# maxgreat/Instance-Search

Hardware: AMD Instinct MI355X
Metric: images/sec descriptor extract + query x gallery search (higher is better)
Workload: dtype f32; 1 GPU; BASELINE configs[1]: ResNet-50 fully-conv global descriptors + top-100 cosine search, 10000-row gallery shard per GPU, 224x224 synthetic images; gallery_rows_per_gpu=10000, descriptor_dim=2048, k=100, backbone=resnet50, backbone_dtype=f32, activation_layout=NHWC, bn_folded=True, parallelism=gallery-row shards x1 + DP extraction, ranks=1

## Files before the change

include/isx.h:

```cpp
#ifndef ISX_H_
#define ISX_H_

#include <stddef.h>
#include <stdint.h>

#ifdef __cplusplus
extern "C" {
#endif

#define ISX_CONV_CHUNK 64

#define ISX_OK 0
#define ISX_ERR_ARG (-1)
#define ISX_ERR_WORKSPACE (-2)
#define ISX_ERR_HIP (-3)

typedef void* isx_stream_t;

const char* isx_last_error(void);
int isx_version(void);


int isx_l2norm_rows(const float* x, int64_t B, int64_t D, float eps, float* y, isx_stream_t stream);

int isx_l2norm_shift_rows(const float* x, const float* shift, int64_t B, int64_t F, float eps, float* y,
                          isx_stream_t stream);

int isx_gap_l2(const float* fmap, int64_t B, int C, int H, int W, float eps, float* y, isx_stream_t stream);

int isx_gap_l2_nhwc(const float* fmap, int64_t B, int C, int H, int W, float eps, float* y, isx_stream_t stream);

int isx_bias_act_inplace(float* y, const float* bias, const float* residual, int64_t n, int C, int64_t inner, int relu,
                         isx_stream_t stream);

int isx_images_u8_to_f32(const uint8_t* img, int64_t B, int H, int W, float mean0, float mean1, float mean2, float std0, float std1,
                         float std2, int channels_last, float* out, isx_stream_t stream);

int isx_bias_relu_maxpool_nhwc(const float* y, const float* bias, int64_t B, int H, int W, int C, float* out, isx_stream_t stream);

int isx_conv3x3_expand_nhwc(const float* x, int64_t B, int H, int W, int Cin, const float* w2_ohwi, const float* b2, int stride,
                            const float* w3t, int Cout, const float* b3, const float* residual, int relu, float* y, isx_stream_t stream);

int isx_conv3x3_expand_dual_nhwc(const float* t, int64_t B, int H, int W, int Cin, const float* w2_ohwi, const float* b2, const float* x2,
                                 const float* wcat_t, int Cout, const float* bias, int relu, float* y, isx_stream_t stream);

int isx_stem7x7_pool_nhwc(const float* x, int64_t B, int H, int W, const float* w_ohwi, const float* bias, float* out,
                          isx_stream_t stream);

int isx_conv1x1_nhwc(const float* x, int64_t M, int Cin, const float* w, int Cout, const float* bias,
                     const float* residual, int relu, float* y, isx_stream_t stream);

int isx_conv1x1_dual_nhwc(const float* t, int K1, const float* x, int64_t B, int H, int W, int K2, int stride, const float* w_cat,
                          int Cout, const float* bias, int relu, float* y, isx_stream_t stream);

int isx_conv3x3_nhwc(const float* x, int64_t B, int H, int W, int Cin, const float* w_ohwi, int Cout, int stride,
                     const float* bias, const float* residual, int relu, float* y, isx_stream_t stream);

int isx_boxpool_s1(const float* fmap, int64_t B, int C, int H, int W, int kh, int kw, float* out,
                   isx_stream_t stream);

int isx_boxpool_s1_nhwc(const float* fmap, int64_t B, int C, int H, int W, int kh, int kw, float* out,
                        isx_stream_t stream);


int isx_best_location_desc(const float* cls, int64_t B, int K, int Hp, int Wp, float eps, float* desc,
                           int64_t* loc, isx_stream_t stream);

int isx_region_topk(const float* cls, int64_t B, int K, int Hp, int Wp, int k, int64_t* flat_idx, float* score,
                    isx_stream_t stream);

int isx_region_gather_l2(const float* fmap, int64_t B, int C, int Hf, int Wf, int kh, int kw, const int64_t* flat_idx, int k,
                         int Wp, const float* shift, float eps, float* rows, isx_stream_t stream);

int isx_best_location_desc_nhwc(const float* cls, int64_t B, int K, int Hp, int Wp, float eps, float* desc,
                                int64_t* loc, isx_stream_t stream);
int isx_region_topk_nhwc(const float* cls, int64_t B, int K, int Hp, int Wp, int k, int64_t* flat_idx, float* score,
                         isx_stream_t stream);
// ... 145 lines not shown
```

instance-search_amd/csrc/conv.hip:

```cpp
#include <stdlib.h>

#include "conv3x3_tile.hpp"

namespace isx {

template <int TM, int TN, int BK, int CHUNK = kConvChunk, bool POSMAJ = false>
__device__ __forceinline__ void conv3x3_tile(float* __restrict__ lds, const float* __restrict__ x, int64_t M, const float* __restrict__ Wt, int64_t N,
                                             const Conv3x3Geom& g, float* __restrict__ C, int64_t m0, int64_t n0,
                                             const float* __restrict__ bias, const float* __restrict__ res, int relu, const float* __restrict__ mask = nullptr) {
    f32x16 acc[TM][TN];
    if constexpr (POSMAJ) {
        if (pos_major_tile(g, M, m0).b0 >= M / (g.Ho * g.Wo)) return;
    }
    conv3x3_mainloop<TM, TN, BK, false, CHUNK, POSMAJ>(lds, x, M, Wt, N, g, m0, n0, acc);
    const int lane = threadIdx.x & 63, wave = threadIdx.x >> 6;
    const int wm_u = __builtin_amdgcn_readfirstlane(wave >> 1), wn_u = __builtin_amdgcn_readfirstlane(wave & 1);
    if constexpr (POSMAJ) {
        const PosMajorTile pt = pos_major_tile(g, M, m0);
        const int64_t off = (int64_t)pt.p * N, ldc = (int64_t)g.Ho * g.Wo * N;
        conv_epilogue_buffers<TM, TN, TM * TN < 4 ? 1 : 2>(acc, C + off, res ? res + off : nullptr, bias, relu, pt.b0, pt.B, n0, N, ldc, 64 * TM, wm_u * (32 * TM), wn_u * (32 * TN), lane & 31, lane >> 5);
        return;
    }
    conv_epilogue_buffers<TM, TN, (CHUNK == 0 || TM * TN < 4) ? 1 : 2>(acc, C, res, bias, relu, m0, M, n0, N, N, 64 * TM, wm_u * (32 * TM), wn_u * (32 * TN), lane & 31, lane >> 5, mask);
}
// ... 142 lines not shown
}

__global__ __launch_bounds__(256, kWgPerCu128) void conv1x1_dual_tail_kernel(const float* __restrict__ t, const float* __restrict__ x, int64_t M, const float* __restrict__ Wt,
                                                                   int64_t N, DualGeom g, float* __restrict__ C, TileMap tm_big, TileMap tm_small,
                                                                   int64_t m_split, const float* __restrict__ bias, int relu) {
    __shared__ float lds[kTailKernelLdsFloats];
    tail_tile_of_block(tm_big, tm_small, m_split, [&](auto T, auto BK, int64_t m0, int64_t n0) {
        conv1x1_dual_tile<T(), T(), BK()>(lds, t, x, M, Wt, N, g, C, m0, n0, bias, relu);
    });
}

template <int TM, int TN, int BK>
static void launch_dual(const float* t, const float* x, int64_t M, const float* w, int64_t N, const DualGeom& g, float* y, const float* bias, int relu,
                        hipStream_t st) {
    TileMap tm;
    tm.m_active = nullptr;
    tm.tiles_m = (int)((M + 64 * TM - 1) / (64 * TM));
    tm.tiles_n = (int)((N + 64 * TN - 1) / (64 * TN));
    const int64_t split = (TM == 2 && TN == 2) ? gemm_tail_split_rows(M, N, 256 * kWgPerCu128) : 0;
    if (split > 0) {
        const TailGrid tg = gemm_tail_grid(M, N, split);
        hipLaunchKernelGGL(conv1x1_dual_tail_kernel, dim3(tg.blocks), dim3(256), 0, st, t, x, M, w, N, g, y, tg.big, tg.small, split, bias, relu);
        return;
    }
    hipLaunchKernelGGL((conv1x1_dual_nhwc_kernel<TM, TN, BK>), dim3((unsigned)(tm.tiles_m * tm.tiles_n)), dim3(256), 0, st, t, x, M, w, N, g, y, tm,
                       bias, relu);
}

static std::atomic<int> g_force_conv_cfg{[] { const char* e = getenv("ISX_DEBUG_CONV_CFG"); return e ? atoi(e) : -1; }()};
static std::atomic<int> g_pos_major{[] { const char* e = getenv("ISX_DEBUG_CONV_CFG"); return !(e && atoi(e) == 8); }()};

constexpr int kPosMajorMaxP = 28 * 28;

static const float kEff3x3[4] = {0.90f, 0.0f, 0.865f, 0.87f};

}

using namespace isx;

ISX_API int isx_conv1x1_nhwc(const float* x, int64_t M, int Cin, const float* w, int Cout, const float* bias, const float* residual,
                             int relu, float* y, isx_stream_t stream) {
    ISX_REQUIRE(M >= 0 && Cin > 0 && Cout > 0 && Cout <= (1 << 20), "isx_conv1x1_nhwc: bad shape M=%lld Cin=%d Cout=%d (Cout <= 2^20: 32-bit offsets inside a tile's rows)", (long long)M, Cin, Cout);
    if (M == 0) return ISX_OK;
    ISX_REQUIRE(x && w && bias && y, "isx_conv1x1_nhwc: null pointer");
    ISX_REQUIRE(y != x && y != residual, "isx_conv1x1_nhwc: y must not alias x or residual");
    if (g_force_conv_cfg != 9 && conv1x1_stream_applicable(M, Cin, Cout, x, residual))
        return launch_conv1x1_stream(x, M, w, Cin, Cout, bias, residual, relu ? 1 : 0, y, (hipStream_t)stream);
    return launch_conv1x1_gemm(x, M, w, Cout, Cin, y, bias, residual, relu ? 1 : 0, (hipStream_t)stream);
}

ISX_API int isx_conv3x3_nhwc(const float* x, int64_t B, int H, int W, int Cin, const float* w_ohwi, int Cout, int stride,
                             const float* bias, const float* residual, int relu, float* y, isx_stream_t stream) {
    ISX_REQUIRE(B >= 0 && H > 0 && W > 0 && Cin > 0 && Cout > 0 && (stride == 1 || stride == 2),
                "isx_conv3x3_nhwc: bad shape B=%lld H=%d W=%d Cin=%d Cout=%d stride=%d", (long long)B, H, W, Cin, Cout, stride);
    ISX_REQUIRE(Cin % 32 == 0, "isx_conv3x3_nhwc: Cin=%d must be a multiple of 32", Cin);
    ISX_REQUIRE(Cout <= (1 << 20), "isx_conv3x3_nhwc: Cout=%d above 2^20 (32-bit offsets inside a tile's rows)", Cout);
    ISX_REQUIRE(H < 32767 && W < 32767 && B * H * W < (1ll << 31), "isx_conv3x3_nhwc: input has too many pixels for 32-bit pixel indices");
    if (B == 0) return ISX_OK;
    ISX_REQUIRE(x && w_ohwi && bias && y, "isx_conv3x3_nhwc: null pointer");
    ISX_REQUIRE((((uintptr_t)x | (uintptr_t)w_ohwi) % 16) == 0, "isx_conv3x3_nhwc: x and w must be 16-B aligned");
    ISX_REQUIRE(y != x && y != residual, "isx_conv3x3_nhwc: y must not alias x or residual");
    Conv3x3Geom g;
    g.H = H; g.W = W; g.Cin = Cin; g.stride = stride;
    g.Ho = (H - 1) / stride + 1;
    g.Wo = (W - 1) / stride + 1;
    const int64_t M = B * g.Ho * g.Wo, N = Cout;
    ISX_REQUIRE(((M + 63) / 64) * ((N + 63) / 64) < (1ll << 31), "isx_conv3x3_nhwc: too many tiles");
    const int64_t P = (int64_t)g.Ho * g.Wo;
    const bool pos_major = g_pos_major && Cin % kConvChunk == 0 && B >= 128 && P <= kPosMajorMaxP &&
                           (128ll * H * W + 2 * W + 4) * Cin * 4 < (1ll << 32) && 128ll * P * Cout * 4 < (1ll << 31);
    const int64_t Mv = pos_major && ((B + 127) / 128 * P * 2) * ((N + 63) / 64) < (1ll << 31) ? (B + 127) / 128 * P * 128 : 0;
    const int64_t Ms = Mv > 0 ? Mv : M;
    int best = pick_tile_cfg(Ms, N, gemm_tail_split_rows(Ms, N, 256 * kWgPerCu128), kEff3x3, 0xD, kWgPerCu128);
    { const int fc_ = g_force_conv_cfg; if (fc_ == 0 || fc_ == 2 || fc_ == 3) best = fc_; }
    hipStream_t st = (hipStream_t)stream;
    with_tile_shape<0xD>(best, [&](auto TM, auto TN, auto BK) {
        launch_conv3x3<TM(), TN(), BK()>(x, M, w_ohwi, N, g, y, bias, residual, relu ? 1 : 0, st, nullptr, false, Mv);
    });
    ISX_CHECK_LAUNCH("isx_conv3x3_nhwc");
    return ISX_OK;
}

ISX_API int isx_conv3x3_dgrad_nhwc(const float* dz, int64_t B, int H, int W, int Cout, const float* wt, int Cin, const float* mask, float* dx,
                                   isx_stream_t stream) {
    ISX_REQUIRE(B >= 0 && H > 0 && W > 0 && Cin > 0 && Cout > 0, "isx_conv3x3_dgrad_nhwc: bad shape B=%lld H=%d W=%d Cout=%d Cin=%d", (long long)B, H, W, Cout, Cin);
    ISX_REQUIRE(Cout % 32 == 0, "isx_conv3x3_dgrad_nhwc: Cout=%d must be a multiple of 32", Cout);
    ISX_REQUIRE(Cin <= (1 << 20) && H < 32767 && W < 32767 && B * H * W < (1ll << 31), "isx_conv3x3_dgrad_nhwc: shape out of the 32-bit index range");
    if (B == 0) return ISX_OK;
    ISX_REQUIRE(dz && wt && dx, "isx_conv3x3_dgrad_nhwc: null pointer");
    ISX_REQUIRE((((uintptr_t)dz | (uintptr_t)wt) % 16) == 0, "isx_conv3x3_dgrad_nhwc: dz and wt must be 16-B aligned");
    ISX_REQUIRE(dx != dz && dx != mask, "isx_conv3x3_dgrad_nhwc: dx must not alias an input");
    Conv3x3Geom g;
    g.H = H; g.W = W; g.Cin = Cout; g.stride = 1; g.Ho = H; g.Wo = W;
    const int64_t M = B * H * W, N = Cin;
    const int best = pick_tile_cfg(M, N, 0, kEff3x3, 0xD);
    hipStream_t st = (hipStream_t)stream;
    with_tile_shape<0xD>(best, [&](auto TM, auto TN, auto BK) {
        launch_conv3x3<TM(), TN(), BK()>(dz, M, wt, N, g, dx, nullptr, nullptr, 0, st, mask, true);
    });
    ISX_CHECK_LAUNCH("isx_conv3x3_dgrad_nhwc");
    return ISX_OK;
}

ISX_API int isx_conv1x1_dual_nhwc(const float* t, int K1, const float* x, int64_t B, int H, int W, int K2, int stride, const float* w_cat,
// ... 34 lines not shown
```

instance-search_amd/csrc/expand.hip:

```cpp
#include "expand_kernel.hpp"

using namespace isx;

ISX_API int isx_conv3x3_expand_nhwc(const float* x, int64_t B, int H, int W, int Cin, const float* w2_ohwi, const float* b2, int stride,
                                    const float* w3t, int Cout, const float* b3, const float* residual, int relu, float* y, isx_stream_t stream) {
    ISX_REQUIRE(B >= 0 && H > 0 && W > 0 && Cin > 0 && (stride == 1 || stride == 2),
                "isx_conv3x3_expand_nhwc: bad shape B=%lld H=%d W=%d Cin=%d stride=%d", (long long)B, H, W, Cin, stride);
    ISX_REQUIRE(Cin % 32 == 0, "isx_conv3x3_expand_nhwc: Cin=%d must be a multiple of 32", Cin);
    ISX_REQUIRE(Cout == 256, "isx_conv3x3_expand_nhwc: Cout=%d (this kernel is built for 64 mid channels -> 256)", Cout);
    ISX_REQUIRE(H < 32767 && W < 32767 && B * H * W < (1ll << 31), "isx_conv3x3_expand_nhwc: input has too many pixels for 32-bit pixel indices");
    if (B == 0) return ISX_OK;
    ISX_REQUIRE(x && w2_ohwi && b2 && w3t && b3 && y, "isx_conv3x3_expand_nhwc: null pointer");
    ISX_REQUIRE((((uintptr_t)x | (uintptr_t)w2_ohwi | (uintptr_t)w3t) % 16) == 0, "isx_conv3x3_expand_nhwc: x, w2 and w3t must be 16-B aligned");
    ISX_REQUIRE(y != x && y != residual, "isx_conv3x3_expand_nhwc: y must not alias x or residual");
    Conv3x3Geom g;
    g.H = H; g.W = W; g.Cin = Cin; g.stride = stride;
    g.Ho = (H - 1) / stride + 1;
    g.Wo = (W - 1) / stride + 1;
    const int64_t M = B * g.Ho * g.Wo;
    ISX_REQUIRE((M + 63) / 64 < (1ll << 31), "isx_conv3x3_expand_nhwc: too many tiles");
    hipLaunchKernelGGL((conv3x3_expand_kernel<4, false>), dim3((unsigned)((M + 63) / 64)), dim3(256), 0, (hipStream_t)stream, x, M, w2_ohwi, g, b2, w3t, b3, residual,
                       relu ? 1 : 0, y);
    ISX_CHECK_LAUNCH("isx_conv3x3_expand_nhwc");
    return ISX_OK;
}

ISX_API int isx_conv3x3_expand_dual_nhwc(const float* t, int64_t B, int H, int W, int Cin, const float* w2_ohwi, const float* b2, const float* x2,
                                         const float* wcat_t, int Cout, const float* bias, int relu, float* y, isx_stream_t stream) {
    ISX_REQUIRE(B >= 0 && H > 0 && W > 0 && Cin > 0, "isx_conv3x3_expand_dual_nhwc: bad shape B=%lld H=%d W=%d Cin=%d", (long long)B, H, W, Cin);
    ISX_REQUIRE(Cin % 32 == 0, "isx_conv3x3_expand_dual_nhwc: Cin=%d must be a multiple of 32", Cin);
    ISX_REQUIRE(Cout == 256, "isx_conv3x3_expand_dual_nhwc: Cout=%d (this kernel is built for 64 mid channels -> 256)", Cout);
    ISX_REQUIRE(H < 32767 && W < 32767 && B * H * W < (1ll << 31), "isx_conv3x3_expand_dual_nhwc: input has too many pixels for 32-bit pixel indices");
    if (B == 0) return ISX_OK;
    ISX_REQUIRE(t && w2_ohwi && b2 && x2 && wcat_t && bias && y, "isx_conv3x3_expand_dual_nhwc: null pointer");
    ISX_REQUIRE((((uintptr_t)t | (uintptr_t)w2_ohwi | (uintptr_t)wcat_t | (uintptr_t)x2) % 16) == 0, "isx_conv3x3_expand_dual_nhwc: t, x2, w2 and wcat_t must be 16-B aligned");
    ISX_REQUIRE(y != t && y != x2, "isx_conv3x3_expand_dual_nhwc: y must not alias an input");
    Conv3x3Geom g;
    g.H = H; g.W = W; g.Cin = Cin; g.stride = 1; g.Ho = H; g.Wo = W;
    const int64_t M = B * H * W;
    hipLaunchKernelGGL((conv3x3_expand_kernel<4, true>), dim3((unsigned)((M + 63) / 64)), dim3(256), 0, (hipStream_t)stream, t, M, w2_ohwi, g, b2, wcat_t, bias, x2,
                       relu ? 1 : 0, y);
    ISX_CHECK_LAUNCH("isx_conv3x3_expand_dual_nhwc");
    return ISX_OK;
}
```

instance-search_amd/csrc/expand_kernel.hpp:

```cpp
#pragma once
#include "conv3x3_tile.hpp"

namespace isx {

template <int TN2, bool DUAL, bool STAMPS = false>
__global__ __launch_bounds__(256, DUAL ? 2 : 4) void conv3x3_expand_kernel(const float* __restrict__ x, int64_t M, const float* __restrict__ W2, Conv3x3Geom g,
                                                                const float* __restrict__ b2, const float* __restrict__ W3t, const float* __restrict__ b3,
                                                                const float* __restrict__ res, int relu, float* __restrict__ y,
                                                                unsigned long long* __restrict__ stamps = nullptr) {
    constexpr int COUT = 64 * TN2, LDY = 64 + 1, TILE_F = 32 * (64 + 64 + 2 * lds_pad(32));
    __shared__ float lds[(DUAL ? 2 : 1) * TILE_F];
    static_assert(TILE_F >= 64 * LDY, "mid tile must fit the operand stages");
    const int nwg = (int)gridDim.x, b = (int)blockIdx.x;
    const int64_t m0 = (int64_t)xcd_remap(b, nwg) * 64;

    auto stamp = [&](int i) { if (STAMPS && threadIdx.x == 0) stamps[(int64_t)blockIdx.x * 8 + i] = __builtin_amdgcn_s_memtime(); };
    stamp(0);
    float4 x2r[4];
    if (DUAL) {
        const int64_t left = M - m0;
        const auto xr2 = uniform_rsrc(res + m0 * 64, (left < 64 ? left : 64) * 256);
#pragma unroll
        for (int j = 0; j < 4; ++j) x2r[j] = __builtin_bit_cast(float4, __builtin_amdgcn_raw_buffer_load_b128(xr2, (unsigned)((j * 256 + (int)threadIdx.x) * 16), 0, 0));
    }
    f32x16 acc[1][1];
    conv3x3_mainloop<1, 1, 32, true>(lds, x, M, W2, 64, g, m0, 0, acc);
    stamp(1);

    const int lane = threadIdx.x & 63, wave = threadIdx.x >> 6;
    const int wm = wave >> 1, wn = wave & 1, l31 = lane & 31, half = lane >> 5;
    if (DUAL) {
#pragma unroll
        for (int j = 0; j < 4; ++j) {
// ... 33 lines not shown
#pragma unroll
                for (int e = 0; e < 16; ++e) acc3[i][j][e] = 0.0f;
    }
#pragma unroll
    for (int s = 0; s < (DUAL ? 64 : 32); ++s) {
        const int ao = s < 32 ? 2 * s * LDY : TILE_F + 2 * (s - 32) * LDY;
        const float a0 = a_base[ao], a1 = a_base[ao + 32];
        float bq[NJ];
#pragma unroll
        for (int j = 0; j < NJ; ++j)
            bq[j] = __builtin_bit_cast(float, __builtin_amdgcn_raw_buffer_load_b32(wr, wvo, wso + (unsigned)((2 * s * COUT + 32 * j) * 4), 0));
#pragma unroll
        for (int j = 0; j < NJ; ++j) {
            if (DUAL && s >= 32) {
                acc3[0][j] = __builtin_amdgcn_mfma_f32_32x32x2f32(a0, bq[j], acc3[0][j], 0, 0, 0);
                acc3[1][j] = __builtin_amdgcn_mfma_f32_32x32x2f32(a1, bq[j], acc3[1][j], 0, 0, 0);
            } else {
                acc2[0][j] = __builtin_amdgcn_mfma_f32_32x32x2f32(a0, bq[j], acc2[0][j], 0, 0, 0);
                acc2[1][j] = __builtin_amdgcn_mfma_f32_32x32x2f32(a1, bq[j], acc2[1][j], 0, 0, 0);
            }
        }
    }
    if (DUAL) {
#pragma unroll
        for (int i = 0; i < 2; ++i)
#pragma unroll
            for (int j = 0; j < NJ; ++j) acc2[i][j] = acc2[i][j] + acc3[i][j];
    }
    stamp(3);
    conv_epilogue_buffers<2, NJ, 2>(acc2, y, DUAL ? nullptr : res, b3, relu, m0, M, 0, COUT, COUT, 64, 0, wave_u * (32 * NJ), l31, half);
    if (STAMPS) { asm volatile("s_waitcnt vmcnt(0)" ::: "memory"); stamp(4); }
}

}
```

instance-search_amd/csrc/isx_internal.hpp:

```cpp
#pragma once
#include <atomic>

#include "isx_common.hpp"

namespace isx {

constexpr int kEpiScores = 0, kEpiFilter = 1, kEpiConv = 2, kEpiMaskedGrad = 3;
template <int EPI> struct EpiArgs {};
template <> struct EpiArgs<kEpiFilter> { const float* thr; uint8_t* gflag; int ngrp; };
template <> struct EpiArgs<kEpiConv> { const float* bias; const float* residual; int relu; };
template <> struct EpiArgs<kEpiMaskedGrad> { const float* mask; const float* add; };
using ScoresArgs = EpiArgs<kEpiScores>;
using FilterArgs = EpiArgs<kEpiFilter>;
using ConvArgs = EpiArgs<kEpiConv>;
using MaskedGradArgs = EpiArgs<kEpiMaskedGrad>;

int launch_cosine_gemm(const float* Q, int64_t M, const float* G, int64_t N, int D, float* C, int64_t ldc,
                       hipStream_t st, const int* m_active = nullptr);

int launch_cosine_gemm_filter(const float* Q, int64_t M, const float* G, int64_t N, int D, float* C, int64_t ldc,
                              const float* thr, uint8_t* gflag, hipStream_t st, const int* m_active = nullptr);

int launch_conv1x1_gemm(const float* x, int64_t M, const float* w, int64_t N, int D, float* y, const float* bias, const float* residual, int relu,
                        hipStream_t st);

int launch_gemm_masked(const float* A, int64_t M, const float* Bt, int64_t N, int D, float* C, const float* mask, const float* add, hipStream_t st);

extern std::atomic<int> g_tail_split;
int64_t gemm_tail_split_rows(int64_t M, int64_t N, int64_t slots = 1024);
struct TileMap {
    int tiles_m, tiles_n;
    const int* m_active;
};
struct TailGrid { TileMap big, small; unsigned blocks; };
TailGrid gemm_tail_grid(int64_t rows, int64_t N, int64_t split);
int pick_tile_cfg(int64_t M, int64_t N, int64_t split, const float* eff, unsigned mask, int wg_per_cu_128 = 4);

bool conv1x1_stream_applicable(int64_t M, int Cin, int Cout, const float* x, const float* res);
int launch_conv1x1_stream(const float* x, int64_t M, const float* w, int Cin, int Cout, const float* bias, const float* res, int relu, float* y,
                          hipStream_t st);

int launch_gemm_f16(const _Float16* Q, int64_t M, const _Float16* G, int64_t N, int D, float* C, int64_t ldc, const float* thr,
                    uint8_t* gflag, hipStream_t st);

int launch_select(const float* sim, int64_t M, int64_t Nc, int64_t ld, int64_t col_base, int k, uint64_t* carry,
                  bool first, bool emit, int64_t idx_base, float* top_score, int64_t* top_idx, hipStream_t st,
                  float* thr_out = nullptr);

int launch_select_groups(const float* sim, const uint8_t* gflag, int64_t M, int64_t Nc, int64_t ld, int64_t col_base, int k,
                         uint64_t* carry, float* thr, int mode, int64_t idx_base, float* top_score, int64_t* top_idx,
                         hipStream_t st, const int* m_active = nullptr, const int* row_map = nullptr, const float* win = nullptr, int k_win = 0);

constexpr int kGroupSelectMaxK = 256;

constexpr int kSelectMaxK = 1024;

struct TopkJob {
    const char* who;
    const float* Q; const float* G;
    const _Float16* Qh; const _Float16* Gh;
    int64_t M, N; int D, k;
    int64_t idx_base; float* top_score; int64_t* top_idx; bool emit;
    void* ws; size_t ws_bytes; hipStream_t st;
    const int* m_active; const int* row_map;
    const float* win; int k_win;
};
int run_topk_chunks(const TopkJob& job);
size_t topk_fixed_bytes(int64_t M, int k);
size_t topk_chunk_bytes(int64_t M, int64_t nc);
int64_t topk_recommended_chunk(int64_t M, int64_t N);
// ... 3 lines not shown
```

instance-search_amd/isx/_lib.py:

```python
import ctypes as C
import os

import torch

_CSRC = os.path.join(os.path.dirname(os.path.dirname(os.path.abspath(__file__))), "csrc")
LIB_PATH = os.environ.get("ISX_LIB") or os.path.join(_CSRC, "libisx.so")

_lib = None

I64, I32, F32, SZ, VP = C.c_int64, C.c_int, C.c_float, C.c_size_t, C.c_void_p

_SIGNATURES = {
    "isx_version": (C.c_int, []),
    "isx_last_error": (C.c_char_p, []),
    "isx_l2norm_rows": (C.c_int, [VP, I64, I64, F32, VP, VP]),
    "isx_l2norm_rows_bwd": (C.c_int, [VP, VP, I64, I64, F32, VP, VP]),
    "isx_l2norm_shift_rows": (C.c_int, [VP, VP, I64, I64, F32, VP, VP]),
    "isx_gap_l2": (C.c_int, [VP, I64, I32, I32, I32, F32, VP, VP]),
    "isx_gap_l2_nhwc": (C.c_int, [VP, I64, I32, I32, I32, F32, VP, VP]),
    "isx_bias_act_inplace": (C.c_int, [VP, VP, VP, I64, I32, I64, I32, VP]),
    "isx_images_u8_to_f32": (C.c_int, [VP, I64, I32, I32, C.c_float, C.c_float, C.c_float, C.c_float, C.c_float, C.c_float, I32, VP, VP]),
    "isx_bias_relu_maxpool_nhwc": (C.c_int, [VP, VP, I64, I32, I32, I32, VP, VP]),
    "isx_conv1x1_nhwc": (C.c_int, [VP, I64, I32, VP, I32, VP, VP, I32, VP, VP]),
    "isx_conv1x1_dual_nhwc": (C.c_int, [VP, I32, VP, I64, I32, I32, I32, I32, VP, I32, VP, I32, VP, VP]),
    "isx_stem7x7_pool_nhwc": (C.c_int, [VP, I64, I32, I32, VP, VP, VP, VP]),
    "isx_conv3x3_expand_nhwc": (C.c_int, [VP, I64, I32, I32, I32, VP, VP, I32, VP, I32, VP, VP, I32, VP, VP]),
    "isx_conv3x3_expand_dual_nhwc": (C.c_int, [VP, I64, I32, I32, I32, VP, VP, VP, VP, I32, VP, I32, VP, VP]),
    "isx_conv3x3_nhwc": (C.c_int, [VP, I64, I32, I32, I32, VP, I32, I32, VP, VP, I32, VP, VP]),
    "isx_boxpool_s1": (C.c_int, [VP, I64, I32, I32, I32, I32, I32, VP, VP]),
    "isx_boxpool_s1_nhwc": (C.c_int, [VP, I64, I32, I32, I32, I32, I32, VP, VP]),
    "isx_best_location_desc": (C.c_int, [VP, I64, I32, I32, I32, F32, VP, VP, VP]),
    "isx_best_location_desc_nhwc": (C.c_int, [VP, I64, I32, I32, I32, F32, VP, VP, VP]),
    "isx_region_topk_nhwc": (C.c_int, [VP, I64, I32, I32, I32, I32, VP, VP, VP]),
    "isx_region_gather_l2_nhwc": (C.c_int, [VP, I64, I32, I32, I32, I32, I32, VP, I32, I32, VP, F32, VP, VP]),
    "isx_region_topk": (C.c_int, [VP, I64, I32, I32, I32, I32, VP, VP, VP]),
    "isx_region_gather_l2": (C.c_int, [VP, I64, I32, I32, I32, I32, I32, VP, I32, I32, VP, F32, VP, VP]),
    "isx_cosine_sim": (C.c_int, [VP, I64, VP, I64, I32, VP, VP]),
    "isx_cosine_topk_workspace": (SZ, [I64, I64, I32, I32]),
    "isx_cosine_topk": (C.c_int, [VP, I64, VP, I64, I32, I32, I64, VP, VP, VP, SZ, VP]),
    "isx_rows_to_f16": (C.c_int, [VP, I64, I32, VP, VP, VP, VP]),
    "isx_cosine_sim_f16": (C.c_int, [VP, I64, VP, I64, I32, VP, VP]),
    "isx_gallery_to_f16": (C.c_int, [VP, I64, I32, VP, VP, VP]),
    "isx_cosine_topk_fast_workspace": (SZ, [I64, I64, I32, I32, I32]),
    "isx_cosine_topk_fast_fallback_offset": (SZ, [I64, I64, I32, I32, I32]),
    "isx_cosine_topk_fast": (C.c_int, [VP, I64, VP, I64, I32, I32, I64, VP, VP, VP, VP, VP, SZ, VP]),
    "isx_topk_rows": (C.c_int, [VP, I64, I64, I32, I64, VP, VP, VP]),
    "isx_rank_full_workspace": (SZ, [I64, I64]),
    "isx_rank_full": (C.c_int, [VP, I64, I64, VP, VP, SZ, VP]),
    "isx_average_precision": (C.c_int, [VP, I64, I64, VP, VP, I32, VP, VP]),
    "isx_average_precision_sim": (C.c_int, [VP, I64, I64, VP, VP, I32, VP, VP]),
    "isx_masked_sums": (C.c_int, [VP, I64, I64, VP, VP, VP, VP]),
    "isx_dba_groups": (C.c_int, [VP, I64, I32, VP, VP, VP, I32, I32, VP, VP]),
    "isx_topk_merge": (C.c_int, [VP, VP, I32, I64, I32, VP, VP, VP]),
    "isx_mine_negatives": (C.c_int, [VP, I64, VP, VP, VP, I64, I32, VP, VP]),
    "isx_mine_negatives_rows": (C.c_int, [VP, I64, I64, I64, VP, VP, VP, I64, I32, VP, VP]),
    "isx_triplet_loss_fwd": (C.c_int, [VP, VP, VP, I64, I32, F32, I32, VP, VP]),
    "isx_triplet_loss_bwd": (C.c_int, [VP, VP, VP, VP, I64, I32, F32, I32, VP, VP, VP, VP]),
    "isx_triplet_loss_bwd_dev": (C.c_int, [VP, VP, VP, VP, I64, I32, F32, VP, I32, VP, VP, VP, VP]),
    "isx_conv1x1_dgrad_nhwc": (C.c_int, [VP, I64, I32, VP, I32, VP, VP, VP, VP]),
    "isx_conv3x3_dgrad_nhwc": (C.c_int, [VP, I64, I32, I32, I32, VP, I32, VP, VP, VP]),
# ... 62 lines not shown
```

instance-search_amd/isx/ops.py:

```python
import torch

from . import _lib
from ._lib import check, lib

EPS = 1e-10


def _stream():
    return torch.cuda.current_stream().cuda_stream


def _on_current_device(t, name):
    if t.device.index != torch.cuda.current_device():
        raise _lib.IsxError("%s lives on %s but the current device is cuda:%d -- wrap the call in torch.cuda.device(%s)"
                            % (name, t.device, torch.cuda.current_device(), t.device.index))


def _f32(t, name):
    if not (isinstance(t, torch.Tensor) and t.is_cuda):
        raise _lib.IsxError("%s must be a CUDA tensor (libisx has no CPU path)" % name)
    if t.dtype != torch.float32:
        raise _lib.IsxError("%s must be float32, got %s" % (name, t.dtype))
    _on_current_device(t, name)
    return t.contiguous()
# ... 259 lines not shown
        rp = residual.data_ptr()
    bp = _f32(bias, "bias").data_ptr()
    _timed("isx_conv3x3_nhwc", 18.0 * B * Ho * Wo * Cin * Cout, 4.0 * (B * H * W * Cin + B * Ho * Wo * Cout * (2 if rp else 1) + 9 * Cin * Cout),
           lambda: check(lib().isx_conv3x3_nhwc(x.data_ptr(), B, H, W, Cin, w.data_ptr(), Cout, stride, bp, rp, 1 if relu else 0, y.data_ptr(),
                                                _stream()), "isx_conv3x3_nhwc"))
    return y


def conv3x3_expand_nhwc(x, w2_ohwi, b2, stride, w3t, b3, residual=None, relu=True):
    if not (x.is_cuda and x.dtype == torch.float32 and x.dim() == 4 and x.is_contiguous(memory_format=torch.channels_last)):
        raise _lib.IsxError("x must be a channels-last float32 CUDA tensor (B,C,H,W)")
    _on_current_device(x, "x")
    B, Cin, H, W = x.shape
    w2 = _f32(w2_ohwi, "w2_ohwi")
    w3 = _f32(w3t, "w3t")
    if tuple(w2.shape) != (64, 3, 3, Cin) or w3.dim() != 2 or w3.shape[0] != 64:
        raise _lib.IsxError("w2_ohwi must be (64, 3, 3, Cin) and w3t (64, Cout)")
    Cout = w3.shape[1]
    Ho, Wo = (H - 1) // stride + 1, (W - 1) // stride + 1
    y = torch.empty((B, Cout, Ho, Wo), device=x.device, dtype=torch.float32, memory_format=torch.channels_last)
    rp = 0
    if residual is not None:
        if residual.shape != y.shape or residual.dtype != torch.float32 or not residual.is_contiguous(memory_format=torch.channels_last):
            raise _lib.IsxError("residual must be a channels-last float32 tensor of the output's shape")
        rp = residual.data_ptr()
    b2p, b3p = _f32(b2, "b2").data_ptr(), _f32(b3, "b3").data_ptr()
    _timed("isx_conv3x3_expand_nhwc", 2.0 * B * Ho * Wo * (9 * Cin * 64 + 64 * Cout),
           4.0 * (B * H * W * Cin + B * Ho * Wo * Cout * (2 if rp else 1) + 9 * Cin * 64 + 64 * Cout),
           lambda: check(lib().isx_conv3x3_expand_nhwc(x.data_ptr(), B, H, W, Cin, w2.data_ptr(), b2p, stride, w3.data_ptr(), Cout, b3p, rp,
                                                       1 if relu else 0, y.data_ptr(), _stream()), "isx_conv3x3_expand_nhwc"))
    return y


def conv3x3_expand_dual_nhwc(t, w2_ohwi, b2, x2, wcat_t, bias, relu=True):
    for a, n in ((t, "t"), (x2, "x2")):
        if not (a.is_cuda and a.dtype == torch.float32 and a.dim() == 4 and a.is_contiguous(memory_format=torch.channels_last)):
            raise _lib.IsxError("%s must be a channels-last float32 CUDA tensor (B,C,H,W)" % n)
        _on_current_device(a, n)
    B, Cin, H, W = t.shape
    w2 = _f32(w2_ohwi, "w2_ohwi")
    wc = _f32(wcat_t, "wcat_t")
    if tuple(w2.shape) != (64, 3, 3, Cin) or tuple(x2.shape) != (B, 64, H, W) or wc.dim() != 2 or wc.shape[0] != 128:
        raise _lib.IsxError("w2_ohwi must be (64, 3, 3, Cin), x2 (B, 64, H, W) and wcat_t (128, Cout)")
    Cout = wc.shape[1]
    y = torch.empty((B, Cout, H, W), device=t.device, dtype=torch.float32, memory_format=torch.channels_last)
    b2p, bp = _f32(b2, "b2").data_ptr(), _f32(bias, "bias").data_ptr()
    _timed("isx_conv3x3_expand_nhwc", 2.0 * B * H * W * (9 * Cin * 64 + 128 * Cout),
           4.0 * (B * H * W * (Cin + 64 + Cout) + 9 * Cin * 64 + 128 * Cout),
           lambda: check(lib().isx_conv3x3_expand_dual_nhwc(t.data_ptr(), B, H, W, Cin, w2.data_ptr(), b2p, x2.data_ptr(), wc.data_ptr(), Cout, bp,
                                                            1 if relu else 0, y.data_ptr(), _stream()), "isx_conv3x3_expand_dual_nhwc"))
    return y


def boxpool_s1(fmap, kh, kw):
    fmap = _f32(fmap, "fmap")
    B, Cc, H, W = fmap.shape
    out = torch.empty((B, Cc, H - kh + 1, W - kw + 1), device=fmap.device, dtype=torch.float32)
    check(lib().isx_boxpool_s1(fmap.data_ptr(), B, Cc, H, W, kh, kw, out.data_ptr(), _stream()), "isx_boxpool_s1")
    return out


def _is_nhwc(t):
    return t.dim() == 4 and not t.is_contiguous() and t.is_contiguous(memory_format=torch.channels_last)


def boxpool_s1_applicable_nhwc(fmap):
# ... 521 lines not shown
```

instance-search_amd/model/nn_utils.py:

```python
import os

import torch
import torch.nn as nn

from isx import backbones as models


def set_untrained_blocks(containers, n):
    params_of = lambda m: list(m.parameters())
    for seq in containers:
        for m in seq:
            for p in params_of(m):
                p.requires_grad = n >= 0
    frozen = 0
    for seq in containers:
        for m in seq:
            if frozen >= n:
                break
            ps = params_of(m)
            if not ps:
                continue
            for p in ps:
                p.requires_grad = False
            frozen += 1
# ... 187 lines not shown

    def w3t(self):
        wl = self.convs[-1].conv.weight
        if self.downsample is not None:
            wd = self.downsample.conv.weight
            return _derived(self, '_c_w3t', (wl, wd), lambda: self.w_cat().t().contiguous())
        return _derived(self, '_c_w3t', (wl,), lambda: wl.detach().reshape(wl.shape[0], -1).t().contiguous())

    def _fusable_projection(self, x):
        last, d = self.convs[-1], self.downsample
        return (_GEMM_1X1 and _FUSE_PROJECTION and d is not None and last._pointwise() and d.conv.kernel_size == (1, 1) and d.conv.padding == (0, 0)
                and d.conv.groups == 1 and d.conv.stride in ((1, 1), (2, 2)) and last.conv.in_channels % 32 == 0 and d.conv.in_channels % 32 == 0
                and x.is_cuda and x.dtype == torch.float32 and not torch.is_grad_enabled() and x.dim() == 4
                and x.is_contiguous(memory_format=torch.channels_last) and not x.is_contiguous())

    def _fusable_expand_dual(self):
        if not (_FUSE_EXPAND and _IMPLICIT_GEMM_3X3 and len(self.convs) == 3):
            return False
        c2, c3, d = self.convs[1].conv, self.convs[2].conv, self.downsample.conv
        return (c2.kernel_size == (3, 3) and c2.padding == (1, 1) and c2.groups == 1 and c2.dilation == (1, 1) and c2.stride == (1, 1)
                and c2.out_channels == 64 and c2.in_channels % 32 == 0 and self.convs[1].relu and c3.in_channels == 64 and c3.out_channels == 256
                and d.in_channels == 64 and d.stride == (1, 1))

    def _fusable_expand(self, x):
        if not (_FUSE_EXPAND and _GEMM_1X1 and _IMPLICIT_GEMM_3X3 and self.downsample is None and len(self.convs) == 3):
            return False
        c2, c3 = self.convs[1].conv, self.convs[2].conv
        return (c2.kernel_size == (3, 3) and c2.padding == (1, 1) and c2.groups == 1 and c2.dilation == (1, 1) and c2.stride in ((1, 1), (2, 2))
                and c2.out_channels == 64 and c2.in_channels % 32 == 0 and self.convs[1].relu and self.convs[2]._pointwise() and c3.in_channels == 64
                and c3.out_channels == 256 and x.shape[1] == 256 and c2.stride == (1, 1)
                and x.is_cuda and x.dtype == torch.float32 and not torch.is_grad_enabled() and x.dim() == 4
                and x.is_contiguous(memory_format=torch.channels_last) and not x.is_contiguous())

    def forward(self, x):
        if self._fusable_projection(x):
            from isx import ops
            last, d = self.convs[-1], self.downsample
            if self._fusable_expand_dual():
                c2 = self.convs[1]
                t = self.convs[0](x)
                if not t.is_contiguous(memory_format=torch.channels_last):
                    t = t.contiguous(memory_format=torch.channels_last)
                return ops.conv3x3_expand_dual_nhwc(t, c2.w_ohwi(), c2.bias, x, self.w3t(), last.bias, last.relu)
            t = x
            for c in self.convs[:-1]:
                t = c(t)
            if not t.is_contiguous(memory_format=torch.channels_last):
                t = t.contiguous(memory_format=torch.channels_last)
            return ops.conv1x1_dual_nhwc(t, x, self.w_cat(), last.bias, d.conv.stride[0], last.relu)
        if self._fusable_expand(x):
            from isx import ops
            c2, c3 = self.convs[1], self.convs[2]
            t = self.convs[0](x)
            if not t.is_contiguous(memory_format=torch.channels_last):
                t = t.contiguous(memory_format=torch.channels_last)
            return ops.conv3x3_expand_nhwc(t, c2.w_ohwi(), c2.bias, c2.conv.stride[0], self.w3t(), c3.bias, x, c3.relu)
        idt = x if self.downsample is None else self.downsample(x)
        y = x
        for c in self.convs[:-1]:
            y = c(y)
        return self.convs[-1](y, idt)


class _ChannelsLastEntry(nn.Module):

    def forward(self, x):
        if x.is_cuda and x.dim() == 4 and x.dtype == torch.float32 and not torch.is_grad_enabled():
            return x.contiguous(memory_format=torch.channels_last)
        return x


def fold_batch_norm(features, fuse_epilogues=True):
    import copy
    from torch.nn.utils.fusion import fuse_conv_bn_eval

    def fold_block(b):
        convs = [fuse_conv_bn_eval(copy.deepcopy(getattr(b, c)).eval(), copy.deepcopy(getattr(b, n)).eval())
                 for c, n in (('conv1', 'bn1'), ('conv2', 'bn2'), ('conv3', 'bn3')) if hasattr(b, c)]
        down = None
        if b.downsample is not None:
            down = fuse_conv_bn_eval(copy.deepcopy(b.downsample[0]).eval(), copy.deepcopy(b.downsample[1]).eval())
        if fuse_epilogues:
            return _FusedBlock(convs, down)
        b = copy.deepcopy(b)
        for i, (c, n) in enumerate((('conv1', 'bn1'), ('conv2', 'bn2'), ('conv3', 'bn3'))):
            if hasattr(b, c):
                setattr(b, c, convs[i])
                setattr(b, n, nn.Identity())
        if down is not None:
# ... 36 lines not shown
```

profiles/summarize_prof.py:

```python
#!/usr/bin/env python3
import collections
import csv
import datetime
import glob
import json
import os
import sys

HERE = os.path.dirname(os.path.abspath(__file__))


def find(d, suffix):
    hits = sorted(glob.glob(os.path.join(d, "**", "*" + suffix), recursive=True))
    if not hits:
        raise SystemExit("no *%s under %s" % (suffix, d))
    return hits[-1]


def is_isx(name):
    return "isx::" in name or "_ZN3isx" in name


def family(name):
    if "conv1x1_stream_kernel" in name or "conv1x1_tail_kernel" in name:
        return "isx_conv1x1_nhwc"
    if "conv1x1_dual_nhwc_kernel" in name or "conv1x1_dual_tail_kernel" in name:
        return "isx_conv1x1_dual_nhwc"
    if "conv3x3_nhwc_kernel" in name or "conv3x3_tail_kernel" in name:
        return "isx_conv3x3_nhwc"
    if "conv3x3_expand_kernel" in name:
        return "isx_conv3x3_expand_nhwc"
    if "stem7x7_pool_kernel" in name:
        return "isx_stem7x7_pool_nhwc"
    if "gap_l2_nhwc_kernel" in name or "gap_l2_kernel" in name:
        return "gap_l2"
    if "cosine_gemm_kernel<" in name:
        args = name.split("cosine_gemm_kernel<", 1)[1].split(">", 1)[0].replace(" ", "").split(",")
        return "isx_conv1x1_nhwc" if args[3] == "2" else "cosine_gemm"
    return None


def one_step(rows, name_key, start_key):
    rows = sorted(rows, key=lambda r: int(r[start_key]))
    idx = [i for i, r in enumerate(rows) if "gap_l2" in r[name_key]]
    if len(idx) < 3:
        raise SystemExit("fewer than three steps in the trace")
    a, b = idx[-3], idx[-2]
    return rows[a + 1:b + 1]


def main():
    tag, run_dir = sys.argv[1], sys.argv[2]
    stats = find(run_dir, "_kernel_stats.csv")
    trace = find(run_dir, "_kernel_trace.csv")
    rows = list(csv.DictReader(open(stats)))
    keep = [r for r in rows if is_isx(r["Name"])]
    others = [r for r in rows if not is_isx(r["Name"])][:12]
    with open(os.path.join(HERE, tag + "_kernel_stats.csv"), "w", newline="") as f:
        w = csv.DictWriter(f, fieldnames=list(rows[0].keys()))
        w.writeheader()
        for r in keep + others:
            r = dict(r)
            r["Name"] = r["Name"][:160]
            w.writerow(r)
# ... 76 lines not shown
```

Baseline: 15650 images/s.

## Fuse 3x3 conv with 1x1 expand for 128-channel bottleneck blocks

Adds a fused kernel for ResNet bottleneck blocks whose 3x3 conv has 128 output channels and stride 1. The 3x3 result tile is kept in LDS and multiplied directly by the 1x1 expand weights, with bias, residual and ReLU applied in the same kernel. The goal is to avoid writing and re-reading the mid activation and to save a launch. The inner loop is software-pipelined, overlapping weight prefetch, output stores and residual loads with the MFMAs. The cost is higher register and LDS pressure, and the 3x3 part is recomputed for each output tile only if Cout tiles were split, which they are not here.

```diff
diff --git a/include/isx.h b/include/isx.h
--- a/include/isx.h
+++ b/include/isx.h
@@ -43,6 +43,9 @@
 
 int isx_conv3x3_expand_dual_nhwc(const float* t, int64_t B, int H, int W, int Cin, const float* w2_ohwi, const float* b2, const float* x2,
                                  const float* wcat_t, int Cout, const float* bias, int relu, float* y, isx_stream_t stream);
+
+int isx_conv3x3_expand128_nhwc(const float* x, int64_t B, int H, int W, int Cin, const float* w2_ohwi, const float* b2, const float* w3t, int Cout,
+                               const float* b3, const float* residual, int relu, float* y, isx_stream_t stream);
 
 int isx_stem7x7_pool_nhwc(const float* x, int64_t B, int H, int W, const float* w_ohwi, const float* bias, float* out,
                           isx_stream_t stream);
diff --git a/instance-search_amd/csrc/conv.hip b/instance-search_amd/csrc/conv.hip
--- a/instance-search_amd/csrc/conv.hip
+++ b/instance-search_amd/csrc/conv.hip
@@ -198,6 +198,13 @@
 
 constexpr int kPosMajorMaxP = 28 * 28;
 
+int64_t conv3x3_pos_major_rows(int64_t B, int H, int W, int Cin, int Ho, int Wo, int64_t Cout, int64_t tiles_n64) {
+    const int64_t P = (int64_t)Ho * Wo;
+    const bool pos_major = g_pos_major && Cin % kConvChunk == 0 && B >= 128 && P <= kPosMajorMaxP &&
+                           (128ll * H * W + 2 * W + 4) * Cin * 4 < (1ll << 32) && 128ll * P * Cout * 4 < (1ll << 31);
+    return pos_major && ((B + 127) / 128 * P * 2) * tiles_n64 < (1ll << 31) ? (B + 127) / 128 * P * 128 : 0;
+}
+
 static const float kEff3x3[4] = {0.90f, 0.0f, 0.865f, 0.87f};
 
 }
@@ -232,10 +239,7 @@
     g.Wo = (W - 1) / stride + 1;
     const int64_t M = B * g.Ho * g.Wo, N = Cout;
     ISX_REQUIRE(((M + 63) / 64) * ((N + 63) / 64) < (1ll << 31), "isx_conv3x3_nhwc: too many tiles");
-    const int64_t P = (int64_t)g.Ho * g.Wo;
-    const bool pos_major = g_pos_major && Cin % kConvChunk == 0 && B >= 128 && P <= kPosMajorMaxP &&
-                           (128ll * H * W + 2 * W + 4) * Cin * 4 < (1ll << 32) && 128ll * P * Cout * 4 < (1ll << 31);
-    const int64_t Mv = pos_major && ((B + 127) / 128 * P * 2) * ((N + 63) / 64) < (1ll << 31) ? (B + 127) / 128 * P * 128 : 0;
+    const int64_t Mv = conv3x3_pos_major_rows(B, H, W, Cin, g.Ho, g.Wo, Cout, (N + 63) / 64);
     const int64_t Ms = Mv > 0 ? Mv : M;
     int best = pick_tile_cfg(Ms, N, gemm_tail_split_rows(Ms, N, 256 * kWgPerCu128), kEff3x3, 0xD, kWgPerCu128);
     { const int fc_ = g_force_conv_cfg; if (fc_ == 0 || fc_ == 2 || fc_ == 3) best = fc_; }
diff --git a/instance-search_amd/csrc/expand.hip b/instance-search_amd/csrc/expand.hip
--- a/instance-search_amd/csrc/expand.hip
+++ b/instance-search_amd/csrc/expand.hip
@@ -43,3 +43,38 @@
     ISX_CHECK_LAUNCH("isx_conv3x3_expand_dual_nhwc");
     return ISX_OK;
 }
+
+static TailGrid expand128_grid(int64_t rows, int64_t split) {
+    TailGrid t;
+    t.big.m_active = t.small.m_active = nullptr;
+    t.big.tiles_n = t.small.tiles_n = 1;
+    t.big.tiles_m = (int)(split > 0 ? split / 128 : (rows + 127) / 128);
+    t.small.tiles_m = (int)(split > 0 ? (rows - split + 63) / 64 : 0);
+    t.blocks = (unsigned)(t.big.tiles_m + t.small.tiles_m);
+    return t;
+}
+
+ISX_API int isx_conv3x3_expand128_nhwc(const float* x, int64_t B, int H, int W, int Cin, const float* w2_ohwi, const float* b2, const float* w3t, int Cout,
+                                       const float* b3, const float* residual, int relu, float* y, isx_stream_t stream) {
+    ISX_REQUIRE(B >= 0 && H > 0 && W > 0 && Cin > 0 && Cout > 0, "isx_conv3x3_expand128_nhwc: bad shape B=%lld H=%d W=%d Cin=%d Cout=%d", (long long)B, H, W, Cin, Cout);
+    ISX_REQUIRE(Cin % kConvChunk == 0, "isx_conv3x3_expand128_nhwc: Cin=%d must be a multiple of %d", Cin, kConvChunk);
+    ISX_REQUIRE(Cout % 128 == 0 && Cout <= (1 << 20), "isx_conv3x3_expand128_nhwc: Cout=%d must be a multiple of 128, at most 2^20", Cout);
+    ISX_REQUIRE(H < 32767 && W < 32767 && B * H * W < (1ll << 31), "isx_conv3x3_expand128_nhwc: input has too many pixels for 32-bit pixel indices");
+    if (B == 0) return ISX_OK;
+    ISX_REQUIRE(x && w2_ohwi && b2 && w3t && b3 && y, "isx_conv3x3_expand128_nhwc: null pointer");
+    ISX_REQUIRE((((uintptr_t)x | (uintptr_t)w2_ohwi | (uintptr_t)w3t) % 16) == 0, "isx_conv3x3_expand128_nhwc: x, w2 and w3t must be 16-B aligned");
+    ISX_REQUIRE(y != x && y != residual, "isx_conv3x3_expand128_nhwc: y must not alias x or residual");
+    Conv3x3Geom g;
+    g.H = H; g.W = W; g.Cin = Cin; g.stride = 1; g.Ho = H; g.Wo = W;
+    const int64_t M = B * H * W;
+    const int64_t Mv = conv3x3_pos_major_rows(B, H, W, Cin, H, W, Cout, 2);
+    const int64_t rows = Mv > 0 ? Mv : M;
+    const TailGrid tg = expand128_grid(rows, gemm_tail_split_rows(rows, 128, 256 * 2));
+    const int64_t split = (int64_t)tg.big.tiles_m * 128;
+    const dim3 grid(tg.blocks), block(256);
+    hipStream_t st = (hipStream_t)stream;
+    if (Mv > 0) hipLaunchKernelGGL(conv3x3_expand128_kernel<true>, grid, block, 0, st, x, M, w2_ohwi, g, b2, w3t, Cout, b3, residual, relu ? 1 : 0, y, tg.big, tg.small, split);
+    else hipLaunchKernelGGL(conv3x3_expand128_kernel<false>, grid, block, 0, st, x, M, w2_ohwi, g, b2, w3t, Cout, b3, residual, relu ? 1 : 0, y, tg.big, tg.small, split);
+    ISX_CHECK_LAUNCH("isx_conv3x3_expand128_nhwc");
+    return ISX_OK;
+}
diff --git a/instance-search_amd/csrc/expand_kernel.hpp b/instance-search_amd/csrc/expand_kernel.hpp
--- a/instance-search_amd/csrc/expand_kernel.hpp
+++ b/instance-search_amd/csrc/expand_kernel.hpp
@@ -1,4 +1,6 @@
 #pragma once
+#include <utility>
+
 #include "conv3x3_tile.hpp"
 
 namespace isx {
@@ -98,4 +100,160 @@
     if (STAMPS) { asm volatile("s_waitcnt vmcnt(0)" ::: "memory"); stamp(4); }
 }
 
-}
+template <int... I, class F>
+__device__ __forceinline__ void static_for_seq(std::integer_sequence<int, I...>, F&& f) { (f(std::integral_constant<int, I>()), ...); }
+template <int N, class F>
+__device__ __forceinline__ void static_for(F&& f) { static_for_seq(std::make_integer_sequence<int, N>(), f); }
+
+constexpr int kW3Ahead = 8;
+constexpr int kExpand128LdsFloats = 128 * (128 + 1);
+template <int TM, int BK, bool POSMAJ>
+__device__ __forceinline__ void conv3x3_expand128_tile(float* __restrict__ lds, const float* __restrict__ x, int64_t M, const float* __restrict__ W2, const Conv3x3Geom& g,
+                                                       const float* __restrict__ b2, const float* __restrict__ W3t, int Cout, const float* __restrict__ b3,
+                                                       const float* __restrict__ res, int relu, float* __restrict__ y, int64_t m0) {
+    constexpr int BM = 64 * TM, LDY = BM + 1;
+    static_assert(BK * (BM + 128 + 2 * lds_pad(BK)) <= 128 * LDY && 128 * LDY <= kExpand128LdsFloats, "operand stages and mid tile share the LDS");
+    int64_t em0 = m0, eM = M, ldc = Cout;
+    if constexpr (POSMAJ) {
+        const PosMajorTile pt = pos_major_tile(g, M, m0);
+        if (pt.b0 >= pt.B) return;
+        const int64_t off = (int64_t)pt.p * Cout;
+        y += off;
+        if (res) res += off;
+        em0 = pt.b0; eM = pt.B; ldc = (int64_t)g.Ho * g.Wo * Cout;
+    }
+    f32x16 acc[TM][2];
+    conv3x3_mainloop<TM, 2, BK, false, kConvChunk, POSMAJ>(lds, x, M, W2, 128, g, m0, 0, acc);
+
+    const int lane = threadIdx.x & 63, wave = threadIdx.x >> 6;
+    const int wm = wave >> 1, wn = wave & 1, l31 = lane & 31, half = lane >> 5;
+    const int wm_u = __builtin_amdgcn_readfirstlane(wm), wn_u = __builtin_amdgcn_readfirstlane(wn);
+    const int row0 = wm_u * (32 * TM), col0 = wn_u * 64;
+    {
+#pragma unroll
+        for (int j = 0; j < 2; ++j) {
+            const int k = wn * 64 + j * 32 + l31;
+            const float b2v = b2[k];
+#pragma unroll
+            for (int i = 0; i < TM; ++i)
+#pragma unroll
+                for (int e = 0; e < 16; ++e)
+                    lds[k * LDY + wm * (32 * TM) + i * 32 + mfma_row_of(e) + 4 * half] = fmaxf(acc[i][j][e] + b2v, 0.0f);
+        }
+    }
+    __syncthreads();
+
+    const float* a_base = lds + half * LDY + wm * (32 * TM) + l31;
+    const auto wr = uniform_rsrc(W3t, (int64_t)128 * Cout * 4);
+    const unsigned wvo = (unsigned)((half * Cout + l31) * 4);
+    const auto rc = conv_tile_rsrc(y, em0, eM, ldc, BM);
+    const auto rr = conv_tile_rsrc(res ? res : y, em0, res ? eM : em0, ldc, BM);
+    const auto br = uniform_rsrc(b3, (int64_t)Cout * 4);
+    const f32x16 zero = {0.f, 0.f, 0.f, 0.f, 0.f, 0.f, 0.f, 0.f, 0.f, 0.f, 0.f, 0.f, 0.f, 0.f, 0.f, 0.f};
+    auto load_b = [&](int n0, int s, int j) {
+        return __builtin_bit_cast(float, __builtin_amdgcn_raw_buffer_load_b32(wr, wvo, (unsigned)((n0 + col0) * 4) + (unsigned)(2 * s) * (unsigned)Cout * 4u + (unsigned)(j * 128), 0));
+    };
+    const unsigned ldc4 = (unsigned)__builtin_amdgcn_readfirstlane((int)(unsigned)(ldc * 4));
+    unsigned lo[TM];
+#pragma unroll
+    for (int i = 0; i < TM; ++i) lo[i] = (unsigned)(((int64_t)(row0 + i * 32 + 4 * half) * ldc + col0 + l31) * 4);
+    constexpr int NV = TM * 2 * 16, PER = NV / 16;
+    float bq[kW3Ahead][2];
+#pragma unroll
+    for (int s = 0; s < kW3Ahead; ++s) {
+#pragma unroll
+        for (int j = 0; j < 2; ++j) bq[s][j] = load_b(0, s, j);
+    }
+    unsigned wso = (unsigned)(col0 * 4) + (unsigned)(2 * kW3Ahead) * (unsigned)Cout * 4u;
+    __builtin_amdgcn_sched_barrier(0);
+    f32x16 acc1[TM][2];
+    zero_tiles(acc1);
+    float rv[TM][2][16], bv[2];
+    for (int n0 = 0; n0 < Cout; n0 += 128) {
+        unsigned lo_st[TM];
+#pragma unroll
+        for (int i = 0; i < TM; ++i) {
+            lo_st[i] = n0 > 0 ? lo[i] : 0x80000000u;
+            asm volatile("" : "+v"(lo_st[i]));
+        }
+        const unsigned so_st = n0 > 0 ? (unsigned)((n0 - 128) * 4) : 0u, so_ld = (unsigned)(n0 * 4);
+        float a[2][TM];
+#pragma unroll
+        for (int i = 0; i < TM; ++i) a[0][i] = a_base[32 * i];
+        static_for<64>([&](auto S) {
+            constexpr int s = S();
+            if (s + 1 < 64) {
+#pragma unroll
+                for (int i = 0; i < TM; ++i) a[(s + 1) & 1][i] = a_base[2 * (s + 1) * LDY + 32 * i];
+            }
+            const float b[2] = {bq[s % kW3Ahead][0], bq[s % kW3Ahead][1]};
+#pragma unroll
+            for (int j = 0; j < 2; ++j)
+                bq[s % kW3Ahead][j] = __builtin_bit_cast(float, __builtin_amdgcn_raw_buffer_load_b32(wr, wvo + (unsigned)(j * 128), wso, 0));
+            wso = s + kW3Ahead + 1 == 64 ? (unsigned)((n0 + 128 + col0) * 4) : wso + 2u * (unsigned)Cout * 4u;
+            asm volatile("" : "+s"(wso));
+            if (s >= 8 && s < 24) {
+#pragma unroll
+                for (int q = 0; q < PER; ++q) {
+                    const int t = (s - 8) * PER + q, i = t / 32, j = (t / 16) % 2, e = t % 16;
+                    const float v = acc1[i][j][e];
+                    __builtin_amdgcn_raw_buffer_store_b32(__builtin_bit_cast(unsigned, v), rc, lo_st[i] + (unsigned)(j * 128), (unsigned)mfma_row_of(e) * ldc4 + so_st, 0);
+                }
+            }
+            if (s >= 36 && s < 52) {
+                if (s == 36) {
+#pragma unroll
+                    for (int j = 0; j < 2; ++j) bv[j] = __builtin_bit_cast(float, __builtin_amdgcn_raw_buffer_load_b32(br, (unsigned)((n0 + col0 + j * 32 + l31) * 4), 0, 0));
+                }
+#pragma unroll
+                for (int q = 0; q < PER; ++q) {
+                    const int t = (s - 36) * PER + q, i = t / 32, j = (t / 16) % 2, e = t % 16;
+                    rv[i][j][e] = __builtin_bit_cast(float, __builtin_amdgcn_raw_buffer_load_b32(rr, lo[i] + (unsigned)(j * 128), (unsigned)mfma_row_of(e) * ldc4 + so_ld, 0));
+                }
+            }
+            __builtin_amdgcn_sched_barrier(0);
+#pragma unroll
+            for (int i = 0; i < TM; ++i)
+#pragma unroll
+                for (int j = 0; j < 2; ++j) {
+                    if (s < 32) acc[i][j] = __builtin_amdgcn_mfma_f32_32x32x2f32(a[s & 1][i], b[j], s == 0 ? zero : acc[i][j], 0, 0, 0);
+                    else acc1[i][j] = __builtin_amdgcn_mfma_f32_32x32x2f32(a[s & 1][i], b[j], s == 32 ? zero : acc1[i][j], 0, 0, 0);
+                }
+        });
+#pragma unroll
+        for (int i = 0; i < TM; ++i)
+#pragma unroll
+            for (int j = 0; j < 2; ++j)
+#pragma unroll
+                for (int e = 0; e < 16; ++e) {
+                    float v = ((0.0f + acc[i][j][e]) + acc1[i][j][e]) + bv[j];
+                    if (res) v += rv[i][j][e];
+                    if (relu) v = fmaxf(v, 0.0f);
+                    acc1[i][j][e] = v;
+                }
+    }
+    unsigned ldc4e = ldc4;
+    asm volatile("" : "+s"(ldc4e));
+#pragma unroll
+    for (int i = 0; i < TM; ++i)
+#pragma unroll
+        for (int j = 0; j < 2; ++j)
+#pragma unroll
+            for (int e = 0; e < 16; ++e) {
+                const float v = acc1[i][j][e];
+                __builtin_amdgcn_raw_buffer_store_b32(__builtin_bit_cast(unsigned, v), rc, lo[i] + (unsigned)(j * 128), (unsigned)mfma_row_of(e) * ldc4e + (unsigned)((Cout - 128) * 4), 0);
+            }
+}
+
+template <bool POSMAJ>
+__global__ __launch_bounds__(256, 2) void conv3x3_expand128_kernel(const float* __restrict__ x, int64_t M, const float* __restrict__ W2, Conv3x3Geom g,
+                                                                   const float* __restrict__ b2, const float* __restrict__ W3t, int Cout, const float* __restrict__ b3,
+                                                                   const float* __restrict__ res, int relu, float* __restrict__ y, TileMap tm_big, TileMap tm_small,
+                                                                   int64_t m_split) {
+    __shared__ float lds[kExpand128LdsFloats];
+    tail_tile_of_block(tm_big, tm_small, m_split, [&](auto T, auto BK, int64_t m0, int64_t) {
+        conv3x3_expand128_tile<T(), BK(), POSMAJ>(lds, x, M, W2, g, b2, W3t, Cout, b3, res, relu, y, m0);
+    });
+}
+
+}
diff --git a/instance-search_amd/csrc/isx_internal.hpp b/instance-search_amd/csrc/isx_internal.hpp
--- a/instance-search_amd/csrc/isx_internal.hpp
+++ b/instance-search_amd/csrc/isx_internal.hpp
@@ -36,6 +36,8 @@
 TailGrid gemm_tail_grid(int64_t rows, int64_t N, int64_t split);
 int pick_tile_cfg(int64_t M, int64_t N, int64_t split, const float* eff, unsigned mask, int wg_per_cu_128 = 4);
 
+int64_t conv3x3_pos_major_rows(int64_t B, int H, int W, int Cin, int Ho, int Wo, int64_t Cout, int64_t tiles_n64);
+
 bool conv1x1_stream_applicable(int64_t M, int Cin, int Cout, const float* x, const float* res);
 int launch_conv1x1_stream(const float* x, int64_t M, const float* w, int Cin, int Cout, const float* bias, const float* res, int relu, float* y,
                           hipStream_t st);
diff --git a/instance-search_amd/isx/_lib.py b/instance-search_amd/isx/_lib.py
--- a/instance-search_amd/isx/_lib.py
+++ b/instance-search_amd/isx/_lib.py
@@ -26,6 +26,7 @@
     "isx_stem7x7_pool_nhwc": (C.c_int, [VP, I64, I32, I32, VP, VP, VP, VP]),
     "isx_conv3x3_expand_nhwc": (C.c_int, [VP, I64, I32, I32, I32, VP, VP, I32, VP, I32, VP, VP, I32, VP, VP]),
     "isx_conv3x3_expand_dual_nhwc": (C.c_int, [VP, I64, I32, I32, I32, VP, VP, VP, VP, I32, VP, I32, VP, VP]),
+    "isx_conv3x3_expand128_nhwc": (C.c_int, [VP, I64, I32, I32, I32, VP, VP, VP, I32, VP, VP, I32, VP, VP]),
     "isx_conv3x3_nhwc": (C.c_int, [VP, I64, I32, I32, I32, VP, I32, I32, VP, VP, I32, VP, VP]),
     "isx_boxpool_s1": (C.c_int, [VP, I64, I32, I32, I32, I32, I32, VP, VP]),
     "isx_boxpool_s1_nhwc": (C.c_int, [VP, I64, I32, I32, I32, I32, I32, VP, VP]),
diff --git a/instance-search_amd/isx/ops.py b/instance-search_amd/isx/ops.py
--- a/instance-search_amd/isx/ops.py
+++ b/instance-search_amd/isx/ops.py
@@ -315,6 +315,34 @@
     return y
 
 
+def conv3x3_expand128_nhwc(x, w2_ohwi, b2, w3t, b3, residual=None, relu=True):
+    if not (x.dtype == torch.float32 and x.dim() == 4):
+        raise _lib.IsxError("x must be a channels-last float32 CUDA tensor (B,C,H,W)")
+    B, Cin, H, W = x.shape
+    if tuple(w2_ohwi.shape) != (128, 3, 3, Cin) or w3t.dim() != 2 or w3t.shape[0] != 128:
+        raise _lib.IsxError("w2_ohwi must be (128, 3, 3, Cin) and w3t (128, Cout)")
+    Cout = w3t.shape[1]
+    if Cin % 64 != 0 or Cout % 128 != 0:
+        raise _lib.IsxError("Cin must be a multiple of 64 and Cout a multiple of 128")
+    if not (x.is_cuda and x.is_contiguous(memory_format=torch.channels_last)):
+        raise _lib.IsxError("x must be a channels-last float32 CUDA tensor (B,C,H,W)")
+    _on_current_device(x, "x")
+    w2 = _f32(w2_ohwi, "w2_ohwi")
+    w3 = _f32(w3t, "w3t")
+    y = torch.empty((B, Cout, H, W), device=x.device, dtype=torch.float32, memory_format=torch.channels_last)
+    rp = 0
+    if residual is not None:
+        if residual.shape != y.shape or residual.dtype != torch.float32 or not residual.is_contiguous(memory_format=torch.channels_last):
+            raise _lib.IsxError("residual must be a channels-last float32 tensor of the output's shape")
+        rp = residual.data_ptr()
+    b2p, b3p, px = _f32(b2, "b2").data_ptr(), _f32(b3, "b3").data_ptr(), B * H * W
+    _timed("isx_conv3x3_expand128_nhwc", 2.0 * px * (9 * Cin * 128 + 128 * Cout),
+           4.0 * (px * Cin + px * Cout * (2 if rp else 1) + 9 * Cin * 128 + 128 * Cout),
+           lambda: check(lib().isx_conv3x3_expand128_nhwc(x.data_ptr(), B, H, W, Cin, w2.data_ptr(), b2p, w3.data_ptr(), Cout, b3p, rp,
+                                                          1 if relu else 0, y.data_ptr(), _stream()), "isx_conv3x3_expand128_nhwc"))
+    return y
+
+
 def conv3x3_expand_dual_nhwc(t, w2_ohwi, b2, x2, wcat_t, bias, relu=True):
     for a, n in ((t, "t"), (x2, "x2")):
         if not (a.is_cuda and a.dtype == torch.float32 and a.dim() == 4 and a.is_contiguous(memory_format=torch.channels_last)):
diff --git a/instance-search_amd/model/nn_utils.py b/instance-search_amd/model/nn_utils.py
--- a/instance-search_amd/model/nn_utils.py
+++ b/instance-search_amd/model/nn_utils.py
@@ -243,6 +243,16 @@
                 and x.is_cuda and x.dtype == torch.float32 and not torch.is_grad_enabled() and x.dim() == 4
                 and x.is_contiguous(memory_format=torch.channels_last) and not x.is_contiguous())
 
+    def _fusable_expand128(self, x):
+        if not (_FUSE_EXPAND and _GEMM_1X1 and _IMPLICIT_GEMM_3X3 and self.downsample is None and len(self.convs) == 3):
+            return False
+        c2, c3 = self.convs[1].conv, self.convs[2].conv
+        return (c2.kernel_size == (3, 3) and c2.padding == (1, 1) and c2.groups == 1 and c2.dilation == (1, 1) and c2.stride == (1, 1)
+                and c2.out_channels == 128 and c2.in_channels % 64 == 0 and self.convs[1].relu and self.convs[2]._pointwise() and c3.in_channels == 128
+                and c3.out_channels % 128 == 0 and x.shape[1] == c3.out_channels
+                and x.is_cuda and x.dtype == torch.float32 and not torch.is_grad_enabled() and x.dim() == 4
+                and x.is_contiguous(memory_format=torch.channels_last) and not x.is_contiguous())
+
     def forward(self, x):
         if self._fusable_projection(x):
             from isx import ops
@@ -266,6 +276,13 @@
             if not t.is_contiguous(memory_format=torch.channels_last):
                 t = t.contiguous(memory_format=torch.channels_last)
             return ops.conv3x3_expand_nhwc(t, c2.w_ohwi(), c2.bias, c2.conv.stride[0], self.w3t(), c3.bias, x, c3.relu)
+        if self._fusable_expand128(x):
+            from isx import ops
+            c2, c3 = self.convs[1], self.convs[2]
+            t = self.convs[0](x)
+            if not t.is_contiguous(memory_format=torch.channels_last):
+                t = t.contiguous(memory_format=torch.channels_last)
+            return ops.conv3x3_expand128_nhwc(t, c2.w_ohwi(), c2.bias, self.w3t(), c3.bias, x, c3.relu)
         idt = x if self.downsample is None else self.downsample(x)
         y = x
         for c in self.convs[:-1]:
diff --git a/profiles/summarize_prof.py b/profiles/summarize_prof.py
--- a/profiles/summarize_prof.py
+++ b/profiles/summarize_prof.py
@@ -30,6 +30,8 @@
         return "isx_conv3x3_nhwc"
     if "conv3x3_expand_kernel" in name:
         return "isx_conv3x3_expand_nhwc"
+    if "conv3x3_expand128_kernel" in name:
+        return "isx_conv3x3_expand128_nhwc"
     if "stem7x7_pool_kernel" in name:
         return "isx_stem7x7_pool_nhwc"
     if "gap_l2_nhwc_kernel" in name or "gap_l2_kernel" in name:
```

New measurement: 15980 images/s, median of 6. 1.02x the previous value.
